# JosefAlbers/Phi-3-Vision-MLX

Measured on AMD Instinct MI355X. Metric: decode tokens/sec through generate()'s loop (reference-defined; bare graph replays: device_rate) + prefill ms, Phi-3-Vision bf16 1-image VQA, higher is better.
Workload: dtype bf16; 1 GPU; Phi-3-Vision single 336x336 image VQA (BASELINE configs[1]); 17 crops, 2509 image tokens + 22 text tokens, prompt 2531, B=1 per GPU, greedy, EOS suppressed; parallelism=batch-sharded replicas x1, batch_per_gpu=1, tiny=False

## Files before the change

phi-3-vision-mlx_amd/csrc/p3v_attention.hip:

```cpp
#include <stdlib.h>

#include "p3v_common.h"
#include "p3v_gemv3_body.h"
#include "p3v_dot_f8.h"
#include "p3v_dot_q4.h"

struct AttnP {
  const bf16_t* q; const bf16_t* k_past; const bf16_t* v_past; const bf16_t* k_new; const bf16_t* v_new;
  bf16_t* out; const int32_t* pad_len; const int32_t* d_past; float* ws;
  int B, L, nh, nkv, past, past_t, past_div, new_t, pad_div, causal, split_mode, n_split, new_is_cache;
  float scale;
  int head_group;
  float sc2;
  int q_prescaled;
};

template <int HD>
__global__ void __launch_bounds__(256) k_attn(AttnP p) {
  constexpr int KSTR = HD * 2 + 16;
  constexpr int VSTR = 64 * 2 + 16;
  constexpr int NKS = HD / 32;
  constexpr int NDT = HD / 16;
  constexpr int CPR = HD / 8;
  __shared__ __attribute__((aligned(16))) unsigned char Ks[64 * KSTR];
// ... 1133 lines not shown
  if (p.split_mode && !a->ws) return P3V_ERR_ARG;
  if (!p.split_mode) p.n_split = 1;
  hipStream_t s = (hipStream_t)stream;
  if (!p.split_mode && a->L > P3V_DECODE_MAX_L && !p3v_tuning().attn_old)
    return a->hd == 96 ? launch_attn_prefill<96>(p, s) : launch_attn_prefill<64>(p, s);
  dim3 grid(p.split_mode ? p.n_split : p3v_cdiv(a->L, 64), a->n_heads, a->B);
  if (a->hd == 96) hipLaunchKernelGGL(k_attn<96>, grid, dim3(256), 0, s, p);
  else hipLaunchKernelGGL(k_attn<64>, grid, dim3(256), 0, s, p);
  P3V_CHECK_LAUNCH();
  if (p.split_mode) {
    hipLaunchKernelGGL(k_attn_combine2, dim3(a->B * a->n_heads * a->L), dim3(combine_threads(a->n_split)), 0, s, a->ws, a->out, a->L, a->n_heads,
                       a->hd, p.n_split);
    P3V_CHECK_LAUNCH();
  }
  return P3V_OK;
}

struct AttnDecP {
  const bf16_t* qkv; const float* cos_t; const float* sin_t; bf16_t* k_cache; bf16_t* v_cache;
  const int32_t* pad_len; const int32_t* d_past; float* ws;
  int B, L, nh, nkv, past, cache_t, rope_bstride, n_split;
  float scale;
  int chunk, grp, grp_magic;
  int merge;
  bf16_t* out;
  const void* o_w;
  const void* o_sb;
  bf16_t* o_x;
  bf16_t* o_rearm;
  int o_n;
  int fo_remap;
};

#define WS_SENTINEL 0xffffffffu
#ifdef P3V_ATTN_TIMING
__device__ long long p3v_tbuf[8192 * 16];
#define TMARK(k) do { if (threadIdx.x == 0) p3v_tbuf[(blockIdx.x + gridDim.x * blockIdx.y) * 16 + (k)] = wall_clock64(); } while (0)
#define TVAL(k, v) do { if (threadIdx.x == 0) p3v_tbuf[(blockIdx.x + gridDim.x * blockIdx.y) * 16 + (k)] = (v); } while (0)
extern "C" int p3v_timing_read(long long* out, int n) {
  return hipMemcpyFromSymbol(out, HIP_SYMBOL(p3v_tbuf), sizeof(long long) * n) == hipSuccess ? 0 : -1;
}
#else
#define TMARK(k)
#define TVAL(k, v)
#endif
__device__ __forceinline__ void st_wt(float* p, float v) { __hip_atomic_store(p, v, __ATOMIC_RELAXED, __HIP_MEMORY_SCOPE_AGENT); }
__device__ __forceinline__ float ld_wt(const float* p) { return __hip_atomic_load(p, __ATOMIC_RELAXED, __HIP_MEMORY_SCOPE_AGENT); }
__device__ __forceinline__ bool is_sentinel(float v) { return __builtin_bit_cast(uint32_t, v) == WS_SENTINEL; }
typedef float f32x2_t __attribute__((ext_vector_type(2)));
__device__ __forceinline__ void st_wt4(void* p, f32x4_t v) { asm volatile("global_store_dwordx4 %0, %1, off sc1" ::"v"(p), "v"(v) : "memory"); }
__device__ __forceinline__ void st_wt2(void* p, f32x2_t v) { asm volatile("global_store_dwordx2 %0, %1, off sc1" ::"v"(p), "v"(v) : "memory"); }

#define SPLIT_MERGE_SCRATCH(NT) ((NT) / 64 * 130 + 2)
template <int NT>
__device__ __forceinline__ void split_merge(float* base0, bf16_t* out0, size_t out_qstride, int L, int n_split,
                                            const float* own, float* scratch, bool wt_out = false) {
  constexpr int HD = 96, G = NT / 64;
  float* pm = scratch;
  float* pl = scratch + G;
  float (*part)[128] = (float (*)[128])(scratch + 2 * G);
  int* s_timeout = (int*)(scratch + 2 * G + G * 128);
  const int t = threadIdx.x, grp = t >> 6, d0 = t & 63;
  const size_t sstr = (size_t)16 * (HD + 2);
  const bool two = d0 + 64 < HD;
  const float sentinel = __builtin_bit_cast(float, WS_SENTINEL);
  if (t == 0) *s_timeout = 0;
  __syncthreads();
  for (int q = 0; q < L; ++q) {
    float* base = base0 + (size_t)q * (HD + 2);
    const float* own_q = own ? own + q * (HD + 2) : nullptr;
    const int n_glob = own_q ? n_split - 1 : n_split;
    float m, l, a0, a1;
    auto fold = [&](float ms, float ls, float o0, float o1) {
      const float mn = fmaxf(m, ms);
      const float mu = mn == -INFINITY ? 0.f : mn;
      const float ca = __builtin_amdgcn_exp2f(m - mu), cb = __builtin_amdgcn_exp2f(ms - mu);
      float lb = ls * cb, b0 = o0 * cb, b1 = o1 * cb;
      asm volatile("" : "+v"(lb), "+v"(b0), "+v"(b1));
      l = __builtin_fmaf(l, ca, lb);
      a0 = __builtin_fmaf(a0, ca, b0);
      a1 = __builtin_fmaf(a1, ca, b1);
      m = mn;
    };
    constexpr int UB = 6;
    for (unsigned tries = 0;; ++tries) {
      m = -INFINITY, l = 0.f, a0 = 0.f, a1 = 0.f;
      bool bad = false;
      for (int s = grp; s < n_glob; s += UB * G) {
        float ms[UB], ls[UB], o0[UB], o1[UB];
#pragma unroll
        for (int j = 0; j < UB; ++j) {
          const float* r = base + (size_t)min(s + j * G, n_glob - 1) * sstr;
          ms[j] = ld_wt(r + HD); ls[j] = ld_wt(r + HD + 1);
          o0[j] = ld_wt(r + d0); o1[j] = two ? ld_wt(r + d0 + 64) : 0.f;
        }
#pragma unroll
        for (int j = 0; j < UB; ++j) {
          if (s + j * G < n_glob) {
            bad |= is_sentinel(ms[j]) | is_sentinel(ls[j]) | is_sentinel(o0[j]) | is_sentinel(o1[j]);
            fold(ms[j], ls[j], o0[j], o1[j]);
          }
        }
      }
      if (!__any(bad)) { TVAL(6, (long long)tries); break; }
      if (tries >= (1u << 18)) { *s_timeout = 1; break; }
    }
    TMARK(4);
    if (own_q && grp == (n_split - 1) % G)
      fold(own_q[HD], own_q[HD + 1], own_q[d0], two ? own_q[d0 + 64] : 0.f);
    if (G > 1) {
      __syncthreads();
      if (d0 == 0) { pm[grp] = m; pl[grp] = l; }
      part[grp][d0] = a0;
      if (two) part[grp][d0 + 64] = a1;
      __syncthreads();
      if (wt_out) {
        if (t < HD / 2) {
          const bool poison = *s_timeout != 0;
          float M = pm[0];
#pragma unroll
          for (int k = 1; k < G; ++k) M = fmaxf(M, pm[k]);
          const float Mu = M == -INFINITY ? 0.f : M;
          float acc0 = 0.f, acc1 = 0.f, lsum = 0.f;
#pragma unroll
          for (int k = 0; k < G; ++k) {
            const float c = __builtin_amdgcn_exp2f(pm[k] - Mu);
            acc0 = __builtin_fmaf(c, part[k][2 * t], acc0);
            acc1 = __builtin_fmaf(c, part[k][2 * t + 1], acc1);
            lsum = __builtin_fmaf(c, pl[k], lsum);
          }
          const uint32_t wv = poison ? 0x7fc07fc0u : pack_bf16x2(lsum > 0.f ? acc0 / lsum : 0.f, lsum > 0.f ? acc1 / lsum : 0.f);
          __hip_atomic_store((uint32_t*)(out0 + (size_t)q * out_qstride) + t, wv, __ATOMIC_RELAXED, __HIP_MEMORY_SCOPE_AGENT);
        }
      } else if (t < HD) {
        const bool poison = *s_timeout != 0;
        float M = pm[0];
#pragma unroll
        for (int k = 1; k < G; ++k) M = fmaxf(M, pm[k]);
        const float Mu = M == -INFINITY ? 0.f : M;
        float acc = 0.f, lsum = 0.f;
#pragma unroll
        for (int k = 0; k < G; ++k) {
          const float c = __builtin_amdgcn_exp2f(pm[k] - Mu);
          acc = __builtin_fmaf(c, part[k][t], acc);
          lsum = __builtin_fmaf(c, pl[k], lsum);
        }
        out0[(size_t)q * out_qstride + t] = poison ? (bf16_t)0x7fc0 : f32_to_bf16(lsum > 0.f ? acc / lsum : 0.f);
      }
    } else {
      const float inv = *s_timeout ? __builtin_nanf("") : (l > 0.f ? 1.f / l : 0.f);
      out0[(size_t)q * out_qstride + d0] = f32_to_bf16(a0 * inv);
      if (two) out0[(size_t)q * out_qstride + d0 + 64] = f32_to_bf16(a1 * inv);
    }
    TMARK(5);
    for (int s = grp; s < n_glob; s += G) {
      if ((q & 1) == 0) {
        if (d0 < 24) st_wt4(base + s * sstr + 4 * d0, (f32x4_t){sentinel, sentinel, sentinel, sentinel});
        else if (d0 == 24) st_wt2(base + s * sstr + HD, (f32x2_t){sentinel, sentinel});
      } else {
        st_wt(base + s * sstr + d0, sentinel);
        if (two) st_wt(base + s * sstr + d0 + 64, sentinel);
        if (d0 == 0) { st_wt(base + s * sstr + HD, sentinel); st_wt(base + s * sstr + HD + 1, sentinel); }
      }
    }
  }
}

typedef _Float16 f16x8_t __attribute__((ext_vector_type(8)));
typedef _Float16 f16x4_t __attribute__((ext_vector_type(4)));
typedef _Float16 f16x2_t __attribute__((ext_vector_type(2)));
__device__ __forceinline__ uint32_t pack_f16x2(float lo, float hi) {
  const f16x2_t r = {(_Float16)lo, (_Float16)hi};
  return __builtin_bit_cast(uint32_t, r);
}

struct RopeRaw { u32x4_t x0, x1; float4 c0, c1, s0, s1; };
__device__ __forceinline__ RopeRaw rope_fetch(const bf16_t* head_row, int c, const float* ct, const float* st) {
  constexpr int HALF = 48;
  const int d0 = c * 8, lo = d0 < HALF, tb = lo ? d0 : d0 - HALF;
  RopeRaw r;
  r.x0 = *(const u32x4_t*)(head_row + d0);
  r.x1 = *(const u32x4_t*)(head_row + (lo ? d0 + HALF : d0 - HALF));
  r.c0 = *(const float4*)(ct + tb); r.c1 = *(const float4*)(ct + tb + 4);
  r.s0 = *(const float4*)(st + tb); r.s1 = *(const float4*)(st + tb + 4);
  return r;
}
template <bool F16 = false>
__device__ __forceinline__ u32x4_t rope_apply(const RopeRaw& r, int c, unsigned sh16 = 16, unsigned himask = 0xffff0000u) {
  auto bf16lo = [&](unsigned x) { return __builtin_bit_cast(float, x << sh16); };
  auto bf16hi = [&](unsigned x) { return __builtin_bit_cast(float, x & himask); };
  const float cs[8] = {r.c0.x, r.c0.y, r.c0.z, r.c0.w, r.c1.x, r.c1.y, r.c1.z, r.c1.w};
  const float sn[8] = {r.s0.x, r.s0.y, r.s0.z, r.s0.w, r.s1.x, r.s1.y, r.s1.z, r.s1.w};
  const float sg = c < 6 ? -1.f : 1.f;
  u32x4_t o;
#pragma unroll
  for (int j = 0; j < 4; ++j) {
    const float v0 = bf16lo(r.x0[j]) * cs[2 * j] + sg * bf16lo(r.x1[j]) * sn[2 * j];
    const float v1 = bf16hi(r.x0[j]) * cs[2 * j + 1] + sg * bf16hi(r.x1[j]) * sn[2 * j + 1];
    o[j] = F16 ? pack_f16x2(v0, v1) : pack_bf16x2(v0, v1);
  }
  return o;
}

template <bool F16 = false>
__device__ __forceinline__ u32x4_t rope_chunk(const bf16_t* head_row, int c, const float* ct, const float* st) {
  constexpr int HALF = 48;
  const int d0 = c * 8, lo = d0 < HALF;
  const u32x4_t x0 = *(const u32x4_t*)(head_row + d0);
  const u32x4_t x1 = *(const u32x4_t*)(head_row + (lo ? d0 + HALF : d0 - HALF));
// ... 176 lines not shown
    }
    l_run = rows_sum(l_t);
    m_run = m_new;
    DBG_T(5);
    const u32x2_t pw = {pack_bf16x2(s[0], s[1]), pack_bf16x2(s[2], s[3])};
    const s16x4_t pf = __builtin_bit_cast(s16x4_t, pw);
#pragma unroll
    for (int d = 0; d < NDT; ++d) {
      const s16x4_t vf = *(const s16x4_t*)(vtile + v_rd + d * 16 * 128);
      o[d] = __builtin_amdgcn_mfma_f32_16x16x16bf16_1k(vf, pf, o[d], 0, 0, 0);
    }
    DBG_T(6);
  }

  asm volatile("s_waitcnt vmcnt(0) lgkmcnt(0)" ::: "memory");
  __syncthreads();
  if (qvalid) {
    float* Ow = (float*)wreg + qi * HD;
#pragma unroll
    for (int d = 0; d < NDT; ++d) *(f32x4_t*)(Ow + 16 * d + 4 * g) = o[d];
    if (g == 0) { Ml[wave][qi][0] = m_run; Ml[wave][qi][1] = l_run; }
  }
  __syncthreads();
#pragma unroll 1
  for (int idx = tid; idx < n_vnew; idx += 256) {
    const int q = idx / HD, d = idx - q * HD;
    float mk[4], M = -INFINITY;
#pragma unroll
    for (int k = 0; k < 4; ++k) { mk[k] = Ml[k][q][0]; M = fmaxf(M, mk[k]); }
    const float Mu = M == -INFINITY ? 0.f : M;
    float acc = 0.f, lsum = 0.f;
#pragma unroll
    for (int k = 0; k < 4; ++k) {
      const float c = __builtin_amdgcn_exp2f(mk[k] - Mu);
      acc += c * ((const float*)(KV + k * WREG))[q * HD + d];
      lsum += c * Ml[k][q][1];
    }
    float* w = p.ws + ((((size_t)b * p.nh + head) * p.n_split + bx) * 16 + q) * (HD + 2);
    st_wt(w + d, acc);
    if (d == 0) { st_wt(w + HD, M); st_wt(w + HD + 1, lsum); }
  }
  DBG_T(7);
  DBG_W(13, false);
  if (p.merge && bx == p.n_split - 1) {
    __shared__ float merge_scratch[SPLIT_MERGE_SCRATCH(256)];
    split_merge<256>(p.ws + ((size_t)b * p.nh + head) * p.n_split * 16 * (HD + 2), p.out + (size_t)b * p.L * (p.nh * HD) + head * HD,
                     (size_t)p.nh * HD, p.L, p.n_split, nullptr, merge_scratch);
  }
  DBG_W(11, false);
}

struct FoMap { int bx, by, o_unit, o_unit2; };
__host__ __device__ __forceinline__ bool fo_map_ok(int n_split, int nh, int o_n) { return nh == 32 && o_n == 3072 && n_split >= 13 && n_split * nh <= 768; }
__host__ __device__ __forceinline__ FoMap fo_map(int L, int n_split, int nh, int n_units, bool two_on_last) {
  const int G = n_split * nh, base = G >> 8, r = G & 255;
  const int v = L & 255, slot = L >> 8, ns = base + (v < r ? 1 : 0);
  const int m0 = (base - 1) * 256 + 224;
  FoMap m;
  m.o_unit = m.o_unit2 = -1;
  if (L >= m0 && L < m0 + 32) { m.by = L - m0; m.bx = n_split - 1; return m; }
  const int before = L - m0 < 0 ? 0 : (L - m0 > 32 ? 32 : L - m0);
  const int u = L - before;
  m.by = u / (n_split - 1);
  m.bx = u - m.by * (n_split - 1);
  if (v < 224) {
    const int from_last = ns - 1 - slot;
    const int idx = base >= 2 || two_on_last ? (v >= r ? v - r : (224 - r) + v) : v;
    const int second = 224 + idx < n_units ? 224 + idx : -1;
    if (from_last == 0) { m.o_unit = v; if (two_on_last) m.o_unit2 = second; }
    else if (from_last == 1 && !two_on_last) m.o_unit = second;
  }
  return m;
}

#ifndef P3V_FO_SLEEP
#define P3V_FO_SLEEP 4
#endif
enum { FO_NONE = 0, FO_BF16 = 1, FO_F8 = 2, FO_Q4 = 3 };
struct FoP { const void* o_w; const void* o_scale; bf16_t* o_x; const bf16_t* out; int nh; };
template <int KIND, int NU = 1>
__device__ __forceinline__ void fo_project(const FoP f, const int o_wl, unsigned char* lds, const int o_wl2 = -1) {
  constexpr bool F8 = KIND == FO_F8, Q4 = KIND == FO_Q4;
  constexpr int HD = 96, NJ = KIND == FO_BF16 ? 6 : 3;
  const int tid = threadIdx.x, lane = tid & 63, wave = __builtin_amdgcn_readfirstlane(tid >> 6);
  const int Kd = f.nh * HD;
  const size_t row_bytes = (size_t)Kd * (Q4 ? 1 : F8 ? 2 : 4) / 2;
  const bool two = NU > 1 && o_wl2 >= 0;
  int o_u[NU];
  u32x4_t ow[NU][2][Q4 ? 1 : NJ];
  u32x2_t oq[NU][2][Q4 ? 3 : 1];
  uint32_t osb[NU][2][Q4 ? 3 : 1];
  uint32_t ores[NU];
  float osc[NU][2];
#pragma unroll
  for (int k = 0; k < NU; ++k) {
    o_u[k] = (k == 0 ? o_wl : o_wl2) * 4 + wave;
    if (k == 1 && !two) continue;
    const unsigned char* r0p = (const unsigned char*)f.o_w + (size_t)(2 * o_u[k]) * row_bytes;
    if (Q4) {
      const uint32_t* s0 = (const uint32_t*)f.o_scale + (size_t)(2 * o_u[k]) * (Kd / 64) + (lane >> 2);
#pragma unroll
      for (int j = 0; j < 3; ++j) {
        oq[k][0][j] = __builtin_nontemporal_load((const u32x2_t*)r0p + j * 64 + lane);
        oq[k][1][j] = __builtin_nontemporal_load((const u32x2_t*)(r0p + row_bytes) + j * 64 + lane);
        osb[k][0][j] = s0[j * 16];
        osb[k][1][j] = s0[Kd / 64 + j * 16];
      }
    } else {
#pragma unroll
      for (int j = 0; j < NJ; ++j) {
        ow[k][0][j] = __builtin_nontemporal_load((const u32x4_t*)r0p + j * 64 + lane);
        ow[k][1][j] = __builtin_nontemporal_load((const u32x4_t*)(r0p + row_bytes) + j * 64 + lane);
      }
    }
    ores[k] = *(const uint32_t*)(f.o_x + 2 * o_u[k]);
    osc[k][0] = F8 ? ((const float*)f.o_scale)[2 * o_u[k]] : 1.f;
    osc[k][1] = F8 ? ((const float*)f.o_scale)[2 * o_u[k] + 1] : 1.f;
// ... 46 lines not shown
      }
      __syncthreads();
    }
#pragma unroll
    for (int k = 0; k < NU; ++k) {
      if (k == 1 && !two) continue;
      float a0 = 0.f, a1 = 0.f;
      if (Q4) {
#pragma unroll
        for (int j = 0; j < 3; ++j) {
          const int pc = j * 64 + lane;
          const u32x4_t xa = ((const u32x4_t*)xs)[2 * pc], xb = ((const u32x4_t*)xs)[2 * pc + 1];
          const float X = xsum[pc], X128 = 128.f * X;
#pragma unroll
          for (int h = 0; h < 2; ++h) {
            const float D = dot8_q4(oq[k][h][j][1], xb, dot8_q4(oq[k][h][j][0], xa, 0.f));
            const float c = bf16lo(osb[k][h][j]) * (D - X128) + bf16hi(osb[k][h][j]) * X;
            if (h == 0) a0 += c; else a1 += c;
          }
        }
        if (k == 0) TMARK(13);
        a0 = wave_sum(a0);
        a1 = wave_sum(a1);
      } else if (F8) {
#pragma unroll
        for (int j = 0; j < 3; ++j) {
          const u32x4_t xa = ((const u32x4_t*)xs)[2 * (j * 64 + lane)], xb = ((const u32x4_t*)xs)[2 * (j * 64 + lane) + 1];
          a0 = dot16_f8(ow[k][0][j], xa, xb, a0);
          a1 = dot16_f8(ow[k][1][j], xa, xb, a1);
        }
        if (k == 0) TMARK(13);
        a0 = wave_sum(a0) * osc[k][0];
        a1 = wave_sum(a1) * osc[k][1];
      } else {
#pragma unroll
        for (int j = 0; j < 6; ++j) {
          const u32x4_t xa = ((const u32x4_t*)xs)[j * 64 + lane];
          a0 = dot8(ow[k][0][j], xa, a0);
          a1 = dot8(ow[k][1][j], xa, a1);
        }
        if (k == 0) TMARK(13);
        a0 = wave_sum(a0);
        a1 = wave_sum(a1);
      }
      if (lane == 0) {
        const float v0 = bf16lo(ores[k]) + bf16_round(a0), v1 = bf16hi(ores[k]) + bf16_round(a1);
        *(uint32_t*)(f.o_x + 2 * o_u[k]) = timeout ? 0x7fc07fc0u : pack_bf16x2(v0, v1);
      }
    }
    TMARK(14);
  }
}

template <int FO = 0>
__device__ __forceinline__ void attn_decode_body128(const AttnDecP& p, const int bx, const int by, const int bz, unsigned char* KV,
                                                    const int o_unit = -2, const int o_unit2 = -1) {
  constexpr int TK = 128, WK = 32, HD = 96, KROW = HD * 2, VROWB = TK * 2, NKS = 3, NDT = 6, CPR = 12;
  constexpr int KS_BYTES = WK * KROW;
  static_assert(KS_BYTES >= 16 * HD * 4, "a wave's O partial reuses its K slice");
  __shared__ __attribute__((aligned(16))) unsigned char Qs[16 * KROW];
  __shared__ float Ml[4][16][2];
  const int tid = threadIdx.x, lane = tid & 63, g = lane >> 4, qi = lane & 15;
  const int wave = __builtin_amdgcn_readfirstlane(tid >> 6);
  const int b = bz, head = by, kvh = (head * p.grp_magic) >> 16;
  const bool kv_writer = head == kvh * p.grp;
  unsigned char* kslice = KV + wave * KS_BYTES;
  unsigned char* vtile = KV + 4 * KS_BYTES;

  TMARK(0);
#ifdef P3V_ATTN_TIMING
  {
    unsigned hw, xcc;
    asm volatile("s_getreg_b32 %0, hwreg(HW_REG_HW_ID)" : "=s"(hw));
    asm volatile("s_getreg_b32 %0, hwreg(HW_REG_XCC_ID)" : "=s"(xcc));
    TVAL(15, (long long)(((xcc & 15) << 8) | (((hw >> 13) & 7) << 5) | (((hw >> 12) & 1) << 4) | ((hw >> 8) & 15)));
  }
#endif
  int past = p.past, pad = 0;
  const int past_lb = p.past;
  if (p.d_past) asm volatile("s_load_dword %0, %1, 0x0" : "=s"(past) : "s"(p.d_past) : "memory");
  if (p.pad_len) asm volatile("s_load_dword %0, %1, 0x0" : "=s"(pad) : "s"(p.pad_len + b) : "memory");

  const unsigned char* kc = (const unsigned char*)(p.k_cache + ((size_t)b * p.nkv + kvh) * (size_t)p.cache_t * HD);
  bf16_t* vc = p.v_cache + ((size_t)b * p.nkv + kvh) * (size_t)HD * p.cache_t;
  const int kv_lo = bx * TK, kv_hi = min(p.cache_t, kv_lo + TK);
  const size_t vrow = (size_t)p.cache_t * 2;
  auto issue_dma = [&]() {
    const int kv0 = min(kv_lo, p.cache_t - TK);
    const unsigned char* ksrc = kc + (size_t)(kv0 + WK * wave) * KROW;
    const unsigned char* vs = (const unsigned char*)vc + (size_t)kv0 * 2;
    const __amdgpu_buffer_rsrc_t rs_k = __builtin_amdgcn_make_buffer_rsrc((void*)ksrc, 0, 0xffffffff, 0x00020000);
    const __amdgpu_buffer_rsrc_t rs_v = __builtin_amdgcn_make_buffer_rsrc((void*)vs, 0, 0xffffffff, 0x00020000);
#pragma unroll
    for (int j = 0; j < 6; ++j) {
      const int i = j * 64 + lane, r0 = i / CPR, pc = i - r0 * CPR;
      const unsigned koff = r0 * KROW + ((pc ^ ((r0 >> 2) & 3)) << 4);
      __builtin_amdgcn_raw_ptr_buffer_load_lds(rs_k, (dec_lptr_t)(kslice + j * 1024), 16, koff, 0, 0, P3V_ATTN_AUX);
    }
#pragma unroll
    for (int j = 0; j < 6; ++j) {
      const int d = 24 * wave + 4 * j + (lane >> 4);
      const unsigned voff = (unsigned)d * (unsigned)vrow + ((((unsigned)lane & 15) ^ ((unsigned)d & 15)) << 4);
      __builtin_amdgcn_raw_ptr_buffer_load_lds(rs_v, (dec_lptr_t)(vtile + wave * 6144 + j * 1024), 16, voff, 0, 0, P3V_ATTN_AUX);
    }
  };

  const int row_w = (p.nh + 2 * p.nkv) * HD;
// ... 143 lines not shown
    if (!has_new) {
      asm volatile("s_waitcnt vmcnt(0)\n\ts_barrier" ::: "memory");
    }
#pragma unroll
    for (int d = 0; d < NDT; ++d) {
      const u32x2_t a0 = *(const u32x2_t*)(vtile + v_rd[0] + d * 16 * VROWB), a1 = *(const u32x2_t*)(vtile + v_rd[1] + d * 16 * VROWB);
      const u32x4_t aw = {a0[0], a0[1], a1[0], a1[1]};
      o[d] = __builtin_amdgcn_mfma_f32_16x16x32_bf16(__builtin_bit_cast(bf16x8_t, aw), pf, o[d], 0, 0, 0);
    }
  }

  const bool merger = p.merge && bx == p.n_split - 1;
  float* own = (float*)(vtile + 4096);
  static_assert(SPLIT_MERGE_SCRATCH(256) * 4 <= 4096 && 4096 + 16 * (HD + 2) * 4 <= 96 * 256, "merge scratch + own partial fit the V^T tile");
  if (o[0][0] == 12345.f) TVAL(15, 2);
  TMARK(11);
  asm volatile("s_waitcnt vmcnt(0) lgkmcnt(0)" ::: "memory");
  __syncthreads();
  TMARK(2);
  const int o_wl = o_unit != -2 ? o_unit : by * (p.n_split - 1) + bx;
  const bool o_worker = FO && !merger && bx < p.n_split - 1 && o_wl >= 0 && o_wl * 8 < p.o_n;
  if (FO) {
    if (bx == 0 && by == 0) {
      uint32_t* ra = (uint32_t*)p.o_rearm;
      for (int i = tid; i < p.nh * HD / 2; i += 256) ra[i] = 0xffffffffu;
    }
  }
  if (qvalid) {
    float* Ow = (float*)kslice + qi * HD;
#pragma unroll
    for (int d = 0; d < NDT; ++d) *(f32x4_t*)(Ow + 16 * d + 4 * g) = o[d];
    if (g == 0) { Ml[wave][qi][0] = m_run; Ml[wave][qi][1] = l_run; }
  }
  __syncthreads();
#pragma unroll 1
  for (int idx = tid; idx < n_vnew; idx += 256) {
    const int q = idx / HD, d = idx - q * HD;
    float mk[4], M = -INFINITY;
#pragma unroll
    for (int k = 0; k < 4; ++k) { mk[k] = Ml[k][q][0]; M = fmaxf(M, mk[k]); }
    const float Mu = M == -INFINITY ? 0.f : M;
    float acc = 0.f, lsum = 0.f;
#pragma unroll
    for (int k = 0; k < 4; ++k) {
      const float c = __builtin_amdgcn_exp2f(mk[k] - Mu);
      acc += c * ((const float*)(KV + k * KS_BYTES))[q * HD + d];
      lsum += c * Ml[k][q][1];
    }
    if (merger) {
      own[q * (HD + 2) + d] = acc;
      if (d == 0) { own[q * (HD + 2) + HD] = M; own[q * (HD + 2) + HD + 1] = lsum; }
    } else {
      float* w = p.ws + ((((size_t)b * p.nh + head) * p.n_split + bx) * 16 + q) * (HD + 2);
      st_wt(w + d, acc);
      if (d == 0) { st_wt(w + HD, M); st_wt(w + HD + 1, lsum); }
    }
  }
  TMARK(3);
  if (merger)
    split_merge<256>(p.ws + ((size_t)b * p.nh + head) * p.n_split * 16 * (HD + 2), p.out + (size_t)b * p.L * (p.nh * HD) + head * HD,
                     (size_t)p.nh * HD, p.L, p.n_split, own, (float*)vtile, FO != 0);
  if (FO && o_worker) {
    fo_project<FO, 2>(FoP{p.o_w, p.o_sb, p.o_x, p.out, p.nh}, o_wl, KV, o_unit2);
  }
}

__global__ void __launch_bounds__(256) k_attn_decode128(AttnDecP p) {
  __shared__ __attribute__((aligned(1024))) unsigned char KV[4 * 6144 + 96 * 256];
  attn_decode_body128<FO_NONE>(p, blockIdx.x, blockIdx.y, blockIdx.z, KV);
}

__global__ void __launch_bounds__(256) k_attn_decode128_o(AttnDecP p) {
  __shared__ __attribute__((aligned(1024))) unsigned char KV[4 * 6144 + 96 * 256];
  int bx = blockIdx.x, by = blockIdx.y, o_unit = -2, o_unit2 = -1;
  if (p.fo_remap) {
    const FoMap m = fo_map((int)blockIdx.x, p.n_split, p.nh, p.o_n / 8, p.fo_remap == 2);
    bx = m.bx, by = m.by, o_unit = m.o_unit, o_unit2 = m.o_unit2;
  }
  attn_decode_body128<FO_BF16>(p, bx, by, blockIdx.z, KV, o_unit, o_unit2);
}

__global__ void __launch_bounds__(256) k_attn_decode128_o4(AttnDecP p) {
  __shared__ __attribute__((aligned(1024))) unsigned char KV[4 * 6144 + 96 * 256];
  int bx = blockIdx.x, by = blockIdx.y, o_unit = -2, o_unit2 = -1;
  if (p.fo_remap) {
    const FoMap m = fo_map((int)blockIdx.x, p.n_split, p.nh, p.o_n / 8, p.fo_remap == 2);
    bx = m.bx, by = m.by, o_unit = m.o_unit, o_unit2 = m.o_unit2;
  }
  attn_decode_body128<FO_Q4>(p, bx, by, blockIdx.z, KV, o_unit, o_unit2);
}

__global__ void __launch_bounds__(256) k_attn_decode(AttnDecP p) {
  __shared__ __attribute__((aligned(1024))) unsigned char KV[4 * 6144];
  attn_decode_body(p, blockIdx.x, blockIdx.y, blockIdx.z, KV);
}

template <int TK>
__global__ void __launch_bounds__(64) k_attn_decode_stream(AttnDecP p) {
  constexpr int HD = 96, KSTR = HD * 2 + 16, VSTR = TK * 2 + 16, NKS = 3, NDT = 6, CPR = 12;
  constexpr int KIT = TK * CPR / 64, VCH = TK / 8, VIT = HD * VCH / 64;
  __shared__ __attribute__((aligned(16))) unsigned char Ks[TK * KSTR];
  __shared__ __attribute__((aligned(16))) unsigned char Vt[HD * VSTR];
  const int lane = threadIdx.x, g = lane >> 4, qi = lane & 15;
  const int b = blockIdx.z, head = blockIdx.y, kvh = (head * p.grp_magic) >> 16;
  const bool kv_writer = head == kvh * p.grp;
  const float sc2 = p.scale * 1.4426950408889634f;
  const int row_w = (p.nh + 2 * p.nkv) * HD;
  const bf16_t* kc = p.k_cache + ((size_t)b * p.nkv + kvh) * (size_t)p.cache_t * HD;
  bf16_t* vc = p.v_cache + ((size_t)b * p.nkv + kvh) * (size_t)HD * p.cache_t;
  const int chunk = p.chunk;
  const int kv_lo = blockIdx.x * chunk, kv_hi = min(p.cache_t, kv_lo + chunk);

  u32x4_t kreg[KIT], vreg[VIT];
  auto load_tile = [&](int kv0) {
#pragma unroll
    for (int it = 0; it < KIT; ++it) {
      const int i = it * 64 + lane;
      kreg[it] = __builtin_nontemporal_load((const u32x4_t*)(kc + (size_t)(kv0 + i / CPR) * HD + (i % CPR) * 8));
    }
#pragma unroll
    for (int it = 0; it < VIT; ++it) {
      const int i = it * 64 + lane;
      vreg[it] = __builtin_nontemporal_load((const u32x4_t*)(vc + (size_t)(i / VCH) * p.cache_t + kv0 + (i % VCH) * 8));
    }
  };
  if (kv_lo < kv_hi) load_tile(kv_lo);

  const int past = p.d_past ? *p.d_past : p.past;
  const int total = past + p.L;
  const int pad = p.pad_len ? p.pad_len[b] : 0;
  int kv_begin = kv_lo;
  const int kv_end = min(total, kv_hi);
  if (pad > kv_begin) kv_begin = pad & ~(TK - 1);
  const float* cos_b = p.cos_t + (size_t)b * p.rope_bstride * (HD / 2);
  const float* sin_b = p.sin_t + (size_t)b * p.rope_bstride * (HD / 2);

  auto patch_new = [&](int kv0) {
    const int n0 = max(past, kv0), n1 = min(kv_end, kv0 + TK), n_new = n1 - n0;
#pragma unroll 1
    for (int w = lane; w < n_new * CPR; w += 64) {
      const int t = n0 + w / CPR, c = w % CPR, r = t - past;
      const bf16_t* row = p.qkv + ((size_t)b * p.L + r) * row_w;
// ... 208 lines not shown
  int dev = 0;
  hipDeviceProp_t pr;
  if (hipGetDevice(&dev) != hipSuccess || hipGetDeviceProperties(&pr, dev) != hipSuccess) return false;
  return n_heads + (o_n / 8 + 1) / 2 <= pr.multiProcessorCount - 8;
}
template <int KIND>
static int launch_combine_o(const float* ws, void* out, void* o_rearm, const void* o_w, const void* o_sb, void* o_x, int n_heads, int n_split,
                            int o_n, hipStream_t s) {
  const int n_units = o_n / 8, grid_o = n_heads + (n_units + 1) / 2;
  hipLaunchKernelGGL(k_attn_combine_o<KIND>, dim3(grid_o), dim3(combine_threads(n_split)), 0, s, ws, (bf16_t*)out, (bf16_t*)o_rearm, o_w, o_sb,
                     (bf16_t*)o_x, n_heads, n_split, n_units);
  P3V_CHECK_LAUNCH();
  return P3V_OK;
}

__global__ void k_stage_rope(const float* __restrict__ cos_t, const float* __restrict__ sin_t, const int32_t* d_past,
                             int past, float* __restrict__ cos_o, float* __restrict__ sin_o, int L, int tab_t, int half) {
  if (d_past) past = *d_past;
  const int b = blockIdx.x / L, r = blockIdx.x % L;
  for (int i = threadIdx.x; i < half; i += blockDim.x) {
    cos_o[((size_t)b * L + r) * half + i] = cos_t[((size_t)b * tab_t + past + r) * half + i];
    sin_o[((size_t)b * L + r) * half + i] = sin_t[((size_t)b * tab_t + past + r) * half + i];
  }
}

extern "C" int p3v_stage_rope(const float* cos_t, const float* sin_t, int past, const int32_t* d_past, float* cos_out,
                              float* sin_out, int B, int L, int tab_t, int half_dim, void* stream) {
  if (!cos_t || !sin_t || !cos_out || !sin_out || B <= 0 || L <= 0) return P3V_ERR_ARG;
  hipLaunchKernelGGL(k_stage_rope, dim3(B * L), dim3(64), 0, (hipStream_t)stream, cos_t, sin_t, d_past, past, cos_out,
                     sin_out, L, tab_t, half_dim);
  P3V_CHECK_LAUNCH();
  return P3V_OK;
}

#ifdef P3V_ATTN_DEBUG
extern "C" int p3v_debug_read(unsigned long long* out) {
  return hipMemcpyFromSymbol(out, HIP_SYMBOL(p3v_dbg), sizeof(unsigned long long) * 16) == hipSuccess ? 0 : -1;
}
#endif

extern "C" int p3v_attention_decode_can_fuse_oproj(int B, int L, int n_heads, int hd, int n_split, int cache_t, int o_n, int merge_in_launch) {
  if (B != 1 || L != 1 || hd != 96 || n_heads * hd != 3072 || o_n <= 0 || o_n % 8) return 0;
  if (!merge_in_launch)
    return combine_o_ok(B, L, n_heads, hd, n_split, o_n) ? 2 : 0;
  if (!(n_split * 128 >= cache_t && cache_t % 128 == 0 && n_split * 64 < cache_t) || n_split < 2) return 0;
  if ((long)(n_split - 1) * n_heads * 8 < o_n) return 0;
  static long capacity_of[P3V_MAX_DEVICES] = {0};
  int dev = 0;
  if (hipGetDevice(&dev) != hipSuccess || dev < 0 || dev >= P3V_MAX_DEVICES) return 0;
  if (!capacity_of[dev]) {
    int per_cu = 0;
    hipDeviceProp_t pr;
    if (hipGetDeviceProperties(&pr, dev) != hipSuccess) return 0;
    int per_cu4 = 0;
    if (hipOccupancyMaxActiveBlocksPerMultiprocessor(&per_cu, k_attn_decode128_o, 256, 0) != hipSuccess ||
        hipOccupancyMaxActiveBlocksPerMultiprocessor(&per_cu4, k_attn_decode128_o4, 256, 0) != hipSuccess) return 0;
    per_cu = min(per_cu, per_cu4);
    if (per_cu < 1) return 0;
    capacity_of[dev] = (long)per_cu * (pr.multiProcessorCount - 8);
  }
  const long capacity = capacity_of[dev];
  return (long)B * n_heads * n_split <= capacity;
}

extern "C" int p3v_attention_decode_fused_role(int wg, int n_heads, int n_split, int o_n, int map, int* out4) {
  if (!out4 || wg < 0 || n_split < 2 || n_heads < 1 || wg >= n_heads * n_split || (map != 1 && map != 2)) return P3V_ERR_ARG;
  if (!fo_map_ok(n_split, n_heads, o_n)) return P3V_ERR_UNSUPPORTED;
  const FoMap m = fo_map(wg, n_split, n_heads, o_n / 8, map == 2);
  out4[0] = m.bx, out4[1] = m.by, out4[2] = m.o_unit, out4[3] = m.o_unit2;
  return P3V_OK;
}

extern "C" int p3v_attention_decode(const p3v_attn_decode_args_t* a, void* stream) {
  if (!a || !a->qkv || !a->cos_t || !a->sin_t || !a->k_cache || !a->v_cache || !a->out || !a->ws) return P3V_ERR_ARG;
  if (a->hd != 96) return P3V_ERR_UNSUPPORTED;
  if (a->B <= 0 || a->L <= 0 || a->L > P3V_DECODE_MAX_L || a->n_heads % a->n_kv) return P3V_ERR_ARG;
  if (a->n_split < 1 || a->n_split > 128 || a->cache_t % 64) return P3V_ERR_ARG;
  if (((uintptr_t)a->ws | (uintptr_t)a->out) & 15) return P3V_ERR_ARG;
  const int grp = a->n_heads / a->n_kv;
  const int chunk = ((a->cache_t + a->n_split - 1) / a->n_split + 63) & ~63;
  AttnDecP p = {a->qkv, a->cos_t, a->sin_t, a->k_cache, a->v_cache, a->pad_len, a->d_past, a->ws,
                a->B, a->L, a->n_heads, a->n_kv, a->past, a->cache_t, a->rope_bstride, a->n_split, a->scale,
                chunk, grp, (65536 + grp - 1) / grp, a->merge_in_launch, (bf16_t*)a->out,
                a->o_proj_w, a->o_proj_sb, (bf16_t*)a->o_proj_x, (bf16_t*)a->o_rearm, a->o_n, 0};
  hipStream_t s = (hipStream_t)stream;
  dim3 grid(a->n_split, a->n_heads, a->B);
  const int fuse_form = a->o_proj_w ? p3v_attention_decode_can_fuse_oproj(a->B, a->L, a->n_heads, a->hd, a->n_split, a->cache_t, a->o_n, a->merge_in_launch) : 0;
  if (a->o_proj_w && !fuse_form) return P3V_ERR_UNSUPPORTED;
  if (a->o_proj_w && (!a->o_proj_x || !a->o_rearm || ((uintptr_t)a->o_proj_w | (uintptr_t)a->o_proj_x | (uintptr_t)a->o_rearm) & 15)) return P3V_ERR_ARG;
  if (a->o_proj_w && a->o_proj_sb && ((uintptr_t)a->o_proj_sb & 3)) return P3V_ERR_ARG;
  if (fuse_form == 1) {
    if (p3v_tuning().attn_fo_map && fo_map_ok(a->n_split, a->n_heads, a->o_n)) {
      p.fo_remap = p3v_tuning().attn_fo_map;
      grid = dim3(a->n_split * a->n_heads, 1, 1);
    }
    if (a->o_proj_sb) {
      if ((uintptr_t)a->o_proj_sb & 3) return P3V_ERR_ARG;
      hipLaunchKernelGGL(k_attn_decode128_o4, grid, dim3(256), 0, s, p);
    } else {
      hipLaunchKernelGGL(k_attn_decode128_o, grid, dim3(256), 0, s, p);
    }
    P3V_CHECK_LAUNCH();
    return P3V_OK;
  }
  if (a->n_split * 64 >= a->cache_t) hipLaunchKernelGGL(k_attn_decode, grid, dim3(256), 0, s, p);
  else if (a->n_split * 128 >= a->cache_t && a->cache_t % 128 == 0) hipLaunchKernelGGL(k_attn_decode128, grid, dim3(256), 0, s, p);
  else hipLaunchKernelGGL(k_attn_decode_stream<64>, grid, dim3(64), 0, s, p);
  P3V_CHECK_LAUNCH();
  if (a->merge_in_launch) return P3V_OK;
  if (fuse_form == 2)
    return a->o_proj_sb ? launch_combine_o<FO_Q4>(a->ws, a->out, a->o_rearm, a->o_proj_w, a->o_proj_sb, a->o_proj_x, a->n_heads, a->n_split, a->o_n, s)
                        : launch_combine_o<FO_BF16>(a->ws, a->out, a->o_rearm, a->o_proj_w, nullptr, a->o_proj_x, a->n_heads, a->n_split, a->o_n, s);
  hipLaunchKernelGGL(k_attn_combine2, dim3(a->B * a->n_heads * a->L), dim3(combine_threads(a->n_split)), 0, s, a->ws, a->out, a->L, a->n_heads,
                     a->hd, a->n_split);
  P3V_CHECK_LAUNCH();
  return P3V_OK;
}

__global__ void __launch_bounds__(256) k_kv_quantize(const bf16_t* __restrict__ k, const bf16_t* __restrict__ vt,
                                                     uint8_t* __restrict__ k8, uint8_t* __restrict__ v8,
                                                     float* __restrict__ ksc, float* __restrict__ vsc, int hd, int src_t,
                                                     int dst_t, int t0, int n_tok) {
  __shared__ float vmax[64];
  __shared__ bf16_t vtile[96 * 66];
  const int bh = blockIdx.y, tt = blockIdx.x * 64, tid = threadIdx.x, lane = tid & 63, wave = tid >> 6;
  for (int r = wave; r < 64; r += 4) {
    const int t = t0 + tt + r;
    if (tt + r >= n_tok) break;
    const bf16_t* row = k + ((size_t)bh * src_t + t) * hd;
    const float a = lane < hd / 2 ? bf16_to_f32(row[2 * lane]) : 0.f, b = lane < hd / 2 ? bf16_to_f32(row[2 * lane + 1]) : 0.f;
    const float amax = wave_max(fmaxf(fabsf(a), fabsf(b)));
    const float s = amax > 0.f ? amax / 127.f : 1.f, inv = 1.f / s;
    if (lane < hd / 2) {
      const int qa = (int)rintf(a * inv) + 128, qb = (int)rintf(b * inv) + 128;
      *(uint16_t*)(k8 + ((size_t)bh * dst_t + t) * hd + 2 * lane) = (uint16_t)(qa | (qb << 8));
    }
    if (lane == 0) ksc[(size_t)bh * dst_t + t] = s;
  }
  for (int i = tid; i < hd * 64; i += 256) {
    const int d = i >> 6, c = i & 63;
    vtile[d * 66 + c] = tt + c < n_tok ? vt[((size_t)bh * hd + d) * src_t + t0 + tt + c] : (bf16_t)0;
  }
  __syncthreads();
  if (tid < 64) {
    float m = 0.f;
    for (int d = 0; d < hd; ++d) m = fmaxf(m, fabsf(bf16_to_f32(vtile[d * 66 + tid])));
    vmax[tid] = m > 0.f ? m / 127.f : 1.f;
    if (tt + tid < n_tok) vsc[(size_t)bh * dst_t + t0 + tt + tid] = vmax[tid];
  }
  __syncthreads();
  for (int i = tid; i < hd * 64; i += 256) {
    const int d = i >> 6, c = i & 63;
    if (tt + c < n_tok)
// ... 528 lines not shown
  }

  asm volatile("s_waitcnt vmcnt(0) lgkmcnt(0)" ::: "memory");
  __syncthreads();
  if (qvalid) {
    float* Ow = (float*)wreg + qi * HD;
    const float voff = Q8_OFF * p_sum;
#pragma unroll
    for (int d = 0; d < NDT; ++d) *(f32x4_t*)(Ow + 16 * d + 4 * g) = o[d] - voff;
    if (g == 0) { Ml[wave][qi][0] = m_run; Ml[wave][qi][1] = l_run; }
  }
  __syncthreads();
#pragma unroll 1
  for (int idx = tid; idx < n_vnew; idx += 256) {
    const int q = idx / HD, d = idx - q * HD;
    float mk[4], M = -INFINITY;
#pragma unroll
    for (int k = 0; k < 4; ++k) { mk[k] = Ml[k][q][0]; M = fmaxf(M, mk[k]); }
    const float Mu = M == -INFINITY ? 0.f : M;
    float acc = 0.f, lsum = 0.f;
#pragma unroll
    for (int k = 0; k < 4; ++k) {
      const float c = __builtin_amdgcn_exp2f(mk[k] - Mu);
      acc += c * ((const float*)(KV + k * WREG))[q * HD + d];
      lsum += c * Ml[k][q][1];
    }
    float* w = p.ws + ((((size_t)b * p.nh + head) * p.n_split + blockIdx.x) * 16 + q) * (HD + 2);
    st_wt(w + d, acc);
    if (d == 0) { st_wt(w + HD, M); st_wt(w + HD + 1, lsum); }
  }
  if (p.merge && blockIdx.x == p.n_split - 1) {
    __shared__ float merge_scratch[SPLIT_MERGE_SCRATCH(256)];
    split_merge<256>(p.ws + ((size_t)b * p.nh + head) * p.n_split * 16 * (HD + 2), p.out + (size_t)b * p.L * (p.nh * HD) + head * HD,
                     (size_t)p.nh * HD, p.L, p.n_split, nullptr, merge_scratch);
  }
}

template <bool FO>
__global__ void __launch_bounds__(256) k_attn_decode128_q8(AttnDecQ8P p) {
  constexpr int TK = 128, WK = 32, HD = 96, KROWB = HD, VROWB = TK, NKS = 3, NDT = 6, CPR = 12, KROW = HD * 2;
  constexpr int KS_BYTES = WK * KROWB;
  __shared__ __attribute__((aligned(1024))) unsigned char KV[4 * 6144];
  __shared__ __attribute__((aligned(16))) unsigned char Aux[3 * 16 * KROW];
  unsigned char* Qs = Aux;
  unsigned char* Kx = Aux + 16 * KROW;
  unsigned char* Vx = Aux + 2 * 16 * KROW;
  static_assert(SPLIT_MERGE_SCRATCH(256) * 4 <= 2176 && 2176 + 16 * (HD + 2) * 4 <= 3 * 16 * KROW, "merge scratch + own partial fit the aux block");
  __shared__ __attribute__((aligned(16))) float ksl[TK], vsl[TK];
  __shared__ float Ml[4][16][2];
  const int tid = threadIdx.x, lane = tid & 63, g = lane >> 4, qi = lane & 15;
  const int wave = __builtin_amdgcn_readfirstlane(tid >> 6);
  int bx = blockIdx.x, by = blockIdx.y, o_unit = -2, o_unit2 = -1;
  if (FO && p.fo_remap) {
    const FoMap fm = fo_map((int)blockIdx.x, p.n_split, p.nh, p.o_n / 8, p.fo_remap == 2);
    bx = fm.bx, by = fm.by, o_unit = fm.o_unit, o_unit2 = fm.o_unit2;
  }
  const int b = blockIdx.z, head = by, kvh = (head * p.grp_magic) >> 16;
  const bool kv_writer = head == kvh * p.grp;
  unsigned char* kslice = KV + wave * KS_BYTES;
  unsigned char* vtile = KV + 4 * KS_BYTES;
  const size_t bh = (size_t)b * p.nkv + kvh;
  uint8_t* kc = p.k8 + bh * (size_t)p.cache_t * HD;
  uint8_t* vc = p.v8 + bh * (size_t)HD * p.cache_t;
  float* ksc = p.ksc + bh * p.cache_t;
  float* vsc = p.vsc + bh * p.cache_t;

  int past = p.past, pad = 0;
  if (p.d_past) asm volatile("s_load_dword %0, %1, 0x0" : "=s"(past) : "s"(p.d_past) : "memory");
  if (p.pad_len) asm volatile("s_load_dword %0, %1, 0x0" : "=s"(pad) : "s"(p.pad_len + b) : "memory");

  const int kv_lo = bx * TK, kv_hi = min(p.cache_t, kv_lo + TK);
  const int kvd = min(kv_lo, p.cache_t - TK);
  const int row_w = (p.nh + 2 * p.nkv) * HD;
  const int n_vnew = p.L * HD;
  const bf16_t* vnew = p.qkv + (size_t)b * p.L * row_w + (p.nh + p.nkv + kvh) * HD;
  bf16_t v_early = 0;
  if (tid < n_vnew) {
    const unsigned r = (unsigned)tid / HD;
    v_early = vnew[r * (unsigned)row_w + ((unsigned)tid - r * HD)];
  }
  const float scl = tid < TK ? ksc[kvd + tid] : vsc[kvd + tid - TK];
  const float* cos_b = p.cos_t + (size_t)b * p.rope_bstride * (HD / 2);
  const float* sin_b = p.sin_t + (size_t)b * p.rope_bstride * (HD / 2);
  const int tr = tid / CPR, tc = tid - tr * CPR;
  const bool rtask = tr < p.L;
  RopeRaw qraw, kraw;
  if (rtask) {
    const bf16_t* row = p.qkv + ((size_t)b * p.L + tr) * row_w;
    qraw = rope_fetch(row + head * HD, tc, cos_b + tr * (HD / 2), sin_b + tr * (HD / 2));
    kraw = qraw;
    const bf16_t* krow = row + (p.nh + kvh) * HD;
    kraw.x0 = *(const u32x4_t*)(krow + tc * 8);
    kraw.x1 = *(const u32x4_t*)(krow + (tc < 6 ? tc * 8 + 48 : tc * 8 - 48));
  }
  {
    const unsigned char* ksrc = kc + (size_t)(kvd + WK * wave) * KROWB;
    const __amdgpu_buffer_rsrc_t rs_k = __builtin_amdgcn_make_buffer_rsrc((void*)ksrc, 0, 0xffffffff, 0x00020000);
    const __amdgpu_buffer_rsrc_t rs_v = __builtin_amdgcn_make_buffer_rsrc((void*)(vc + kvd), 0, 0xffffffff, 0x00020000);
#pragma unroll
    for (int j = 0; j < 3; ++j)
      __builtin_amdgcn_raw_ptr_buffer_load_lds(rs_k, (dec_lptr_t)(kslice + j * 1024), 16, (unsigned)(j * 1024 + lane * 16), 0, 0, P3V_ATTN_AUX);
#pragma unroll
    for (int j = 0; j < 3; ++j) {
      const int d = 24 * wave + 8 * j + (lane >> 3);
      const unsigned voff = (unsigned)d * (unsigned)p.cache_t + ((((unsigned)lane & 7) ^ ((unsigned)d & 7)) << 4);
      __builtin_amdgcn_raw_ptr_buffer_load_lds(rs_v, (dec_lptr_t)(vtile + wave * 3072 + j * 1024), 16, voff, 0, 0, P3V_ATTN_AUX);
    }
// ... 284 lines not shown
```

phi-3-vision-mlx_amd/csrc/p3v_runtime.hip:

```cpp
#include <ctype.h>
#include <stdlib.h>
#include <string.h>

#include <mutex>

#include "p3v_common.h"

extern "C" int p3v_version(void) { return P3V_VERSION; }

extern "C" const char* p3v_strerror(int code) {
  switch (code) {
    case P3V_OK: return "ok";
    case P3V_ERR_ARG: return "invalid argument (shape, alignment or null pointer)";
    case P3V_ERR_LAUNCH: return "kernel launch failed";
    case P3V_ERR_UNSUPPORTED: return "unsupported combination";
    case P3V_ERR_HIP: return "HIP runtime call failed";
    default: return "unknown error";
  }
}

namespace {
struct Knob { const char* name; int P3vTuning::*field; int dflt; };
const Knob kKnobs[] = {
    {"gemm_big_rows", &P3vTuning::gemm_big_rows, -1},       {"gemm_no_splitk", &P3vTuning::gemm_no_splitk, 0},
    {"gemm_splitk_max_m", &P3vTuning::gemm_splitk_max_m, 1024}, {"gemm_splitk_max_s", &P3vTuning::gemm_splitk_max_s, 8},
    {"gemm_splitk_wgs", &P3vTuning::gemm_splitk_wgs, 256},  {"gemm_128", &P3vTuning::gemm_128, 0},
    {"gemm_persistent", &P3vTuning::gemm_persistent, 1},     {"gemm_no_qkv_fuse", &P3vTuning::gemm_no_qkv_fuse, 0},
    {"gemm_f8_narrow", &P3vTuning::gemm_f8_narrow, -1},     {"attn_no_dma", &P3vTuning::attn_no_dma, 0},
    {"attn_old", &P3vTuning::attn_old, 0},                  {"attn_pp", &P3vTuning::attn_pp, -1},
    {"attn_il", &P3vTuning::attn_il, -1},                   {"attn_il_waves", &P3vTuning::attn_il_waves, -1},
                      {"combine_g", &P3vTuning::combine_g, -1},
    {"kvq_old", &P3vTuning::kvq_old, 0},                    {"q8_old", &P3vTuning::q8_old, 0},
    {"gemv_no_mfma", &P3vTuning::gemv_no_mfma, 0},          {"gemv_no_mfma8", &P3vTuning::gemv_no_mfma8, 0},
    {"gemv_wpc", &P3vTuning::gemv_wpc, 8},                  {"gemv8_wgs", &P3vTuning::gemv8_wgs, 256},
    {"gemv_variant", &P3vTuning::gemv_variant, 3},          {"gemv_rows", &P3vTuning::gemv_rows, 1},
    {"gemv8_min", &P3vTuning::gemv8_min, 2},                {"gemv_mfma8", &P3vTuning::gemv_mfma8, 1},
    {"gemv_f8_wpc", &P3vTuning::gemv_f8_wpc, 16},           {"gemv_q4_wpc", &P3vTuning::gemv_q4_wpc, 8},
    {"gemv_wpw", &P3vTuning::gemv_wpw, 0},                  {"gemv_q4_rows_wgs", &P3vTuning::gemv_q4_rows_wgs, 256},
    {"gemv_q4_rows8", &P3vTuning::gemv_q4_rows8, 1},
    {"gemm_no_skinny", &P3vTuning::gemm_no_skinny, 0},      {"gemm_skinny_max_m", &P3vTuning::gemm_skinny_max_m, 256},
    {"gemm_skinny_s", &P3vTuning::gemm_skinny_s, 0},            {"gemm_skinny_tm128", &P3vTuning::gemm_skinny_tm128, 0},
    {"gemm_rows", &P3vTuning::gemm_rows, 1},
    {"attn_fo_map", &P3vTuning::attn_fo_map, 2},              {"attn_fo_map_q8", &P3vTuning::attn_fo_map_q8, 0},
};
P3vTuning g_tuning;
std::once_flag g_tuning_once;
void tuning_init() {
  for (const Knob& k : kKnobs) {
    char env[64] = "P3V_";
    size_t n = 4;
    for (const char* c = k.name; *c && n + 1 < sizeof(env); ++c) env[n++] = (char)toupper((unsigned char)*c);
    env[n] = 0;
    const char* e = getenv(env);
    g_tuning.*(k.field) = !e ? k.dflt : !strcmp(e, "auto") ? -1 : (*e == 0 ? 1 : atoi(e));
  }
}
}

const P3vTuning& p3v_tuning() {
  std::call_once(g_tuning_once, tuning_init);
  return g_tuning;
}

extern "C" int p3v_set_tuning(const char* name, int value) {
  if (!name) return P3V_ERR_ARG;
  std::call_once(g_tuning_once, tuning_init);
  for (const Knob& k : kKnobs)
    if (!strcmp(k.name, name)) { g_tuning.*(k.field) = value; return P3V_OK; }
  return P3V_ERR_ARG;
}

extern "C" int p3v_get_tuning(const char* name, int* value) {
  if (!name || !value) return P3V_ERR_ARG;
  std::call_once(g_tuning_once, tuning_init);
  for (const Knob& k : kKnobs)
    if (!strcmp(k.name, name)) { *value = g_tuning.*(k.field); return P3V_OK; }
  return P3V_ERR_ARG;
}

extern "C" int p3v_device_props(int device, p3v_props_t* out) {
  if (!out) return P3V_ERR_ARG;
  hipDeviceProp_t pr;
  if (hipGetDeviceProperties(&pr, device) != hipSuccess) return P3V_ERR_HIP;
  memset(out, 0, sizeof(*out));
  out->cu_count = pr.multiProcessorCount;
  out->lds_per_cu = (int)pr.maxSharedMemoryPerMultiProcessor;
  out->wave_size = pr.warpSize;
  out->clock_khz = pr.clockRate;
  out->mem_clock_khz = pr.memoryClockRate;
  out->mem_bus_bits = pr.memoryBusWidth;
  out->hbm_bytes = (int64_t)pr.totalGlobalMem;
  strncpy(out->arch, pr.gcnArchName, sizeof(out->arch) - 1);
  return P3V_OK;
}

extern "C" int p3v_graph_begin(void* stream) {
// ... 44 lines not shown
```

Baseline: 490.9 tokens/s.

## Add map-3 split-decode block remap with plain cached workspace stores

```diff
diff --git a/phi-3-vision-mlx_amd/csrc/p3v_attention.hip b/phi-3-vision-mlx_amd/csrc/p3v_attention.hip
--- a/phi-3-vision-mlx_amd/csrc/p3v_attention.hip
+++ b/phi-3-vision-mlx_amd/csrc/p3v_attention.hip
@@ -1209,7 +1209,7 @@
 __device__ __forceinline__ void st_wt2(void* p, f32x2_t v) { asm volatile("global_store_dwordx2 %0, %1, off sc1" ::"v"(p), "v"(v) : "memory"); }
 
 #define SPLIT_MERGE_SCRATCH(NT) ((NT) / 64 * 130 + 2)
-template <int NT>
+template <int NT, bool XL = false>
 __device__ __forceinline__ void split_merge(float* base0, bf16_t* out0, size_t out_qstride, int L, int n_split,
                                             const float* own, float* scratch, bool wt_out = false) {
   constexpr int HD = 96, G = NT / 64;
@@ -1240,6 +1240,7 @@
       m = mn;
     };
     constexpr int UB = 6;
+    const long long t_wait = XL ? wall_clock64() : 0;
     for (unsigned tries = 0;; ++tries) {
       m = -INFINITY, l = 0.f, a0 = 0.f, a1 = 0.f;
       bool bad = false;
@@ -1260,7 +1261,7 @@
         }
       }
       if (!__any(bad)) { TVAL(6, (long long)tries); break; }
-      if (tries >= (1u << 18)) { *s_timeout = 1; break; }
+      if (tries >= (1u << 18) || (XL && (tries & 15u) == 15u && wall_clock64() - t_wait > 500000)) { *s_timeout = 1; break; }
     }
     TMARK(4);
     if (own_q && grp == (n_split - 1) % G)
@@ -1311,7 +1312,11 @@
     }
     TMARK(5);
     for (int s = grp; s < n_glob; s += G) {
-      if ((q & 1) == 0) {
+      if (XL) {
+        base[s * sstr + d0] = sentinel;
+        if (two) base[s * sstr + d0 + 64] = sentinel;
+        if (d0 == 0) { base[s * sstr + HD] = sentinel; base[s * sstr + HD + 1] = sentinel; }
+      } else if ((q & 1) == 0) {
         if (d0 < 24) st_wt4(base + s * sstr + 4 * d0, (f32x4_t){sentinel, sentinel, sentinel, sentinel});
         else if (d0 == 24) st_wt2(base + s * sstr + HD, (f32x2_t){sentinel, sentinel});
       } else {
@@ -1594,17 +1599,26 @@
 
 struct FoMap { int bx, by, o_unit, o_unit2; };
 __host__ __device__ __forceinline__ bool fo_map_ok(int n_split, int nh, int o_n) { return nh == 32 && o_n == 3072 && n_split >= 13 && n_split * nh <= 768; }
-__host__ __device__ __forceinline__ FoMap fo_map(int L, int n_split, int nh, int n_units, bool two_on_last) {
+__host__ __device__ __forceinline__ FoMap fo_map(int L, int n_split, int nh, int n_units, int map) {
+  const bool two_on_last = map >= 2;
   const int G = n_split * nh, base = G >> 8, r = G & 255;
   const int v = L & 255, slot = L >> 8, ns = base + (v < r ? 1 : 0);
   const int m0 = (base - 1) * 256 + 224;
   FoMap m;
   m.o_unit = m.o_unit2 = -1;
   if (L >= m0 && L < m0 + 32) { m.by = L - m0; m.bx = n_split - 1; return m; }
-  const int before = L - m0 < 0 ? 0 : (L - m0 > 32 ? 32 : L - m0);
-  const int u = L - before;
-  m.by = u / (n_split - 1);
-  m.bx = u - m.by * (n_split - 1);
+  if (map == 3) {
+    const int k = L >> 3, km = m0 >> 3;
+    const int kb = k - (k - km < 0 ? 0 : (k - km > 4 ? 4 : k - km));
+    const int i = kb / (n_split - 1);
+    m.by = (L & 7) + 8 * i;
+    m.bx = kb - i * (n_split - 1);
+  } else {
+    const int before = L - m0 < 0 ? 0 : (L - m0 > 32 ? 32 : L - m0);
+    const int u = L - before;
+    m.by = u / (n_split - 1);
+    m.bx = u - m.by * (n_split - 1);
+  }
   if (v < 224) {
     const int from_last = ns - 1 - slot;
     const int idx = base >= 2 || two_on_last ? (v >= r ? v - r : (224 - r) + v) : v;
@@ -1757,7 +1771,7 @@
   }
 }
 
-template <int FO = 0>
+template <int FO = 0, bool XL = false>
 __device__ __forceinline__ void attn_decode_body128(const AttnDecP& p, const int bx, const int by, const int bz, unsigned char* KV,
                                                     const int o_unit = -2, const int o_unit2 = -1) {
   constexpr int TK = 128, WK = 32, HD = 96, KROW = HD * 2, VROWB = TK * 2, NKS = 3, NDT = 6, CPR = 12;
@@ -2007,13 +2021,18 @@
       if (d == 0) { own[q * (HD + 2) + HD] = M; own[q * (HD + 2) + HD + 1] = lsum; }
     } else {
       float* w = p.ws + ((((size_t)b * p.nh + head) * p.n_split + bx) * 16 + q) * (HD + 2);
-      st_wt(w + d, acc);
-      if (d == 0) { st_wt(w + HD, M); st_wt(w + HD + 1, lsum); }
+      if (XL) {
+        w[d] = acc;
+        if (d == 0) { w[HD] = M; w[HD + 1] = lsum; }
+      } else {
+        st_wt(w + d, acc);
+        if (d == 0) { st_wt(w + HD, M); st_wt(w + HD + 1, lsum); }
+      }
     }
   }
   TMARK(3);
   if (merger)
-    split_merge<256>(p.ws + ((size_t)b * p.nh + head) * p.n_split * 16 * (HD + 2), p.out + (size_t)b * p.L * (p.nh * HD) + head * HD,
+    split_merge<256, XL>(p.ws + ((size_t)b * p.nh + head) * p.n_split * 16 * (HD + 2), p.out + (size_t)b * p.L * (p.nh * HD) + head * HD,
                      (size_t)p.nh * HD, p.L, p.n_split, own, (float*)vtile, FO != 0);
   if (FO && o_worker) {
     fo_project<FO, 2>(FoP{p.o_w, p.o_sb, p.o_x, p.out, p.nh}, o_wl, KV, o_unit2);
@@ -2029,7 +2048,7 @@
   __shared__ __attribute__((aligned(1024))) unsigned char KV[4 * 6144 + 96 * 256];
   int bx = blockIdx.x, by = blockIdx.y, o_unit = -2, o_unit2 = -1;
   if (p.fo_remap) {
-    const FoMap m = fo_map((int)blockIdx.x, p.n_split, p.nh, p.o_n / 8, p.fo_remap == 2);
+    const FoMap m = fo_map((int)blockIdx.x, p.n_split, p.nh, p.o_n / 8, p.fo_remap);
     bx = m.bx, by = m.by, o_unit = m.o_unit, o_unit2 = m.o_unit2;
   }
   attn_decode_body128<FO_BF16>(p, bx, by, blockIdx.z, KV, o_unit, o_unit2);
@@ -2039,10 +2058,22 @@
   __shared__ __attribute__((aligned(1024))) unsigned char KV[4 * 6144 + 96 * 256];
   int bx = blockIdx.x, by = blockIdx.y, o_unit = -2, o_unit2 = -1;
   if (p.fo_remap) {
-    const FoMap m = fo_map((int)blockIdx.x, p.n_split, p.nh, p.o_n / 8, p.fo_remap == 2);
+    const FoMap m = fo_map((int)blockIdx.x, p.n_split, p.nh, p.o_n / 8, p.fo_remap);
     bx = m.bx, by = m.by, o_unit = m.o_unit, o_unit2 = m.o_unit2;
   }
   attn_decode_body128<FO_Q4>(p, bx, by, blockIdx.z, KV, o_unit, o_unit2);
+}
+
+__global__ void __launch_bounds__(256) k_attn_decode128_ox(AttnDecP p) {
+  __shared__ __attribute__((aligned(1024))) unsigned char KV[4 * 6144 + 96 * 256];
+  const FoMap m = fo_map((int)blockIdx.x, p.n_split, p.nh, p.o_n / 8, 3);
+  attn_decode_body128<FO_BF16, true>(p, m.bx, m.by, blockIdx.z, KV, m.o_unit, m.o_unit2);
+}
+
+__global__ void __launch_bounds__(256) k_attn_decode128_o4x(AttnDecP p) {
+  __shared__ __attribute__((aligned(1024))) unsigned char KV[4 * 6144 + 96 * 256];
+  const FoMap m = fo_map((int)blockIdx.x, p.n_split, p.nh, p.o_n / 8, 3);
+  attn_decode_body128<FO_Q4, true>(p, m.bx, m.by, blockIdx.z, KV, m.o_unit, m.o_unit2);
 }
 
 __global__ void __launch_bounds__(256) k_attn_decode(AttnDecP p) {
@@ -2357,10 +2388,12 @@
     int per_cu = 0;
     hipDeviceProp_t pr;
     if (hipGetDeviceProperties(&pr, dev) != hipSuccess) return 0;
-    int per_cu4 = 0;
+    int per_cu4 = 0, per_cux = 0, per_cu4x = 0;
     if (hipOccupancyMaxActiveBlocksPerMultiprocessor(&per_cu, k_attn_decode128_o, 256, 0) != hipSuccess ||
-        hipOccupancyMaxActiveBlocksPerMultiprocessor(&per_cu4, k_attn_decode128_o4, 256, 0) != hipSuccess) return 0;
-    per_cu = min(per_cu, per_cu4);
+        hipOccupancyMaxActiveBlocksPerMultiprocessor(&per_cu4, k_attn_decode128_o4, 256, 0) != hipSuccess ||
+        hipOccupancyMaxActiveBlocksPerMultiprocessor(&per_cux, k_attn_decode128_ox, 256, 0) != hipSuccess ||
+        hipOccupancyMaxActiveBlocksPerMultiprocessor(&per_cu4x, k_attn_decode128_o4x, 256, 0) != hipSuccess) return 0;
+    per_cu = min(min(per_cu, per_cu4), min(per_cux, per_cu4x));
     if (per_cu < 1) return 0;
     capacity_of[dev] = (long)per_cu * (pr.multiProcessorCount - 8);
   }
@@ -2369,9 +2402,9 @@
 }
 
 extern "C" int p3v_attention_decode_fused_role(int wg, int n_heads, int n_split, int o_n, int map, int* out4) {
-  if (!out4 || wg < 0 || n_split < 2 || n_heads < 1 || wg >= n_heads * n_split || (map != 1 && map != 2)) return P3V_ERR_ARG;
+  if (!out4 || wg < 0 || n_split < 2 || n_heads < 1 || wg >= n_heads * n_split || map < 1 || map > 3) return P3V_ERR_ARG;
   if (!fo_map_ok(n_split, n_heads, o_n)) return P3V_ERR_UNSUPPORTED;
-  const FoMap m = fo_map(wg, n_split, n_heads, o_n / 8, map == 2);
+  const FoMap m = fo_map(wg, n_split, n_heads, o_n / 8, map);
   out4[0] = m.bx, out4[1] = m.by, out4[2] = m.o_unit, out4[3] = m.o_unit2;
   return P3V_OK;
 }
@@ -2399,11 +2432,14 @@
       p.fo_remap = p3v_tuning().attn_fo_map;
       grid = dim3(a->n_split * a->n_heads, 1, 1);
     }
+    const bool xl = p.fo_remap == 3;
     if (a->o_proj_sb) {
       if ((uintptr_t)a->o_proj_sb & 3) return P3V_ERR_ARG;
-      hipLaunchKernelGGL(k_attn_decode128_o4, grid, dim3(256), 0, s, p);
+      if (xl) hipLaunchKernelGGL(k_attn_decode128_o4x, grid, dim3(256), 0, s, p);
+      else hipLaunchKernelGGL(k_attn_decode128_o4, grid, dim3(256), 0, s, p);
     } else {
-      hipLaunchKernelGGL(k_attn_decode128_o, grid, dim3(256), 0, s, p);
+      if (xl) hipLaunchKernelGGL(k_attn_decode128_ox, grid, dim3(256), 0, s, p);
+      else hipLaunchKernelGGL(k_attn_decode128_o, grid, dim3(256), 0, s, p);
     }
     P3V_CHECK_LAUNCH();
     return P3V_OK;
@@ -3038,7 +3074,7 @@
   const int wave = __builtin_amdgcn_readfirstlane(tid >> 6);
   int bx = blockIdx.x, by = blockIdx.y, o_unit = -2, o_unit2 = -1;
   if (FO && p.fo_remap) {
-    const FoMap fm = fo_map((int)blockIdx.x, p.n_split, p.nh, p.o_n / 8, p.fo_remap == 2);
+    const FoMap fm = fo_map((int)blockIdx.x, p.n_split, p.nh, p.o_n / 8, p.fo_remap);
     bx = fm.bx, by = fm.by, o_unit = fm.o_unit, o_unit2 = fm.o_unit2;
   }
   const int b = blockIdx.z, head = by, kvh = (head * p.grp_magic) >> 16;
diff --git a/phi-3-vision-mlx_amd/csrc/p3v_runtime.hip b/phi-3-vision-mlx_amd/csrc/p3v_runtime.hip
--- a/phi-3-vision-mlx_amd/csrc/p3v_runtime.hip
+++ b/phi-3-vision-mlx_amd/csrc/p3v_runtime.hip
@@ -41,7 +41,7 @@
     {"gemm_no_skinny", &P3vTuning::gemm_no_skinny, 0},      {"gemm_skinny_max_m", &P3vTuning::gemm_skinny_max_m, 256},
     {"gemm_skinny_s", &P3vTuning::gemm_skinny_s, 0},            {"gemm_skinny_tm128", &P3vTuning::gemm_skinny_tm128, 0},
     {"gemm_rows", &P3vTuning::gemm_rows, 1},
-    {"attn_fo_map", &P3vTuning::attn_fo_map, 2},              {"attn_fo_map_q8", &P3vTuning::attn_fo_map_q8, 0},
+    {"attn_fo_map", &P3vTuning::attn_fo_map, 3},              {"attn_fo_map_q8", &P3vTuning::attn_fo_map_q8, 0},
 };
 P3vTuning g_tuning;
 std::once_flag g_tuning_once;
```

Result: no change. 491.0 tokens/s (median of 4 runs) (+0.0%).
